# zyddnys/manga-image-translator

Hardware: AMD Instinct MI355X
Metric: pages/sec end-to-end (detect+OCR+inpaint), 2048x1456 (higher is better)
Workload: dtype f32

## Files before the change

include/mit_hip.h:

```cpp
#ifndef MIT_HIP_H
#define MIT_HIP_H

#include <stdint.h>

#ifdef __cplusplus
extern "C" {
#endif

#define MIT_ABI_VERSION 25
#define MIT_MAX_TAPS 64

enum MitAct {
    MIT_ACT_NONE = 0,
    MIT_ACT_RELU = 1,
    MIT_ACT_LEAKY = 2,
    MIT_ACT_SILU = 3,
    MIT_ACT_SIGMOID = 4,
    MIT_ACT_GELU = 5
};
#define MIT_ACT_POST_FIRST 0x100

enum MitPad {
    MIT_PAD_ZERO = 0,
    MIT_PAD_REFLECT = 1
};

typedef struct MitTensorMap {
    float *base;
    int64_t zs1, zs0, bs, ys, xs;
    int64_t nhi;
    int32_t nsplit;
    int32_t _pad;
} MitTensorMap;

typedef struct MitConvGemm {
    const float *a;
    int64_t a_zs1, a_zs0, a_bs, a_ys, a_xs;
    int32_t NB, Hi, Wi, Cin;
    int32_t Ho, Wo, sy, sx;
    int32_t ntaps, pad_mode;
    int8_t tap_dy[MIT_MAX_TAPS];
    int8_t tap_dx[MIT_MAX_TAPS];
    int32_t tap_off[MIT_MAX_TAPS];
    const float *w;
    int64_t w_zs1, w_zs0, ldw;
    int32_t Kw, Nw;
    int32_t N;
    int32_t Z, zdiv;
    MitTensorMap c, pre, post;
    const float *scale, *bias;
    int32_t act;
    float act_alpha;
    const uint16_t *w_split;
    int64_t ws_zs0;
    const int32_t *lut_rows;
    const float *lut1, *lut2;
    int64_t lut_ld;
    int32_t nprod;
    int32_t live_img0;
    const int32_t *live_blocks;
    const int32_t *live_start;
    const float *wino_m;
    int64_t wino_zs;
    int32_t wino_n, wino_th, wino_tw;
    int32_t _pad_wino;
} MitConvGemm;

const char *mit_last_error(void);
int mit_abi_version(void);
const char *mit_source_digest(void);

int mit_device_count(int *count);
int mit_device_name(int device, char *buf, int buflen);

int mit_conv_gemm(const MitConvGemm *desc, void *stream);
int mit_conv_gemm_cfg(const MitConvGemm *desc, int cfg, void *stream);
const char *mit_conv_gemm_config_name(int cfg);
int mit_conv_gemm_plan(const MitConvGemm *desc, int cfg, int32_t *tile, int32_t *nb_run);
const char *mit_conv_gemm_config_kernel(int cfg);

int mit_gemm_split_pack(const float *w_dev, int64_t w_zs, int nz, int Kw, int64_t ldw, uint16_t *out_dev, void *stream);
int mit_gemm_mode_set(int mode);
int mit_gemm_mode_get(void);
int64_t mit_gemm_split_min_tiles(int64_t n);

typedef struct MitPGemm {
    const uint16_t *a_planes;
    int64_t a_zs;
    int64_t lda;
    const uint16_t *w_planes;
    int64_t w_zs;
    int64_t ldw;
// ... 217 lines not shown
                        const int64_t *offsets);
int64_t mit_mask_assign_workspace_bytes(int H, int W);
int mit_mask_assign_lines_dev(uint8_t *mask_dev, int H, int W, const int32_t *boxes_xywh_dev, const double *polys_dev,
                              const double *font_size_dev, int M, int V, double keep_threshold, void *ws_dev, int64_t ws_bytes,
                              int32_t *line_rects_dev, void *stream);
int mit_mask_line_crops_dev(const void *ws_dev, int64_t ws_bytes, int H, int W, const int32_t *jobs_dev, const int64_t *offsets_dev,
                            int n_jobs, int64_t total, uint8_t *out_dev, void *stream);
int mit_merge_mask_list(const uint8_t *cands, const int64_t *scores, int n_cands, const uint8_t *pred_mask, int h, int w,
                        int inpaint_dilate, uint8_t *merged);
int mit_otsu_from_hist(const int32_t *hist, int n, int32_t *thresholds);



typedef struct MitXposTables {
    const float *cos_t, *sin_t, *scale_t, *iscale_t;
    int32_t imax, pmax;
} MitXposTables;

typedef struct MitLinear {
    const float *w, *scale, *bias;
    int64_t ldw;
    int32_t K, N, Kp, Np;
    const uint16_t *w_split;
} MitLinear;

typedef struct MitOcrDecoderLayer {
    const float *ln1_w, *ln1_b, *ln2_w, *ln2_b, *ln3_w, *ln3_b;
    MitLinear qkv;
    MitLinear out;
    MitLinear q2;
    MitLinear out2;
    MitLinear ff1, ff2;
} MitOcrDecoderLayer;

typedef struct MitOcr48Decoder {
    MitOcrDecoderLayer layers[5];
    const float *embd;
    MitLinear pred1;
    MitLinear pred;
    MitLinear color1;
    MitLinear color_heads;
    MitXposTables xpos;
    int32_t dict_size, _pad;
} MitOcr48Decoder;

typedef struct MitOcr48DecodeArgs {
    int32_t N, L;
    const float *mem_k;
    const float *mem_v;
    const int32_t *mem_len;
    int32_t max_seq_length;
    int32_t start_tok, end_tok, max_finished, suppress_eos;
    void *workspace;
    int64_t workspace_bytes;
    int32_t *res_tok;
    int32_t *res_len;
    float *res_prob;
    int32_t *res_row;
    float *colors;
    float *trace_logits;
    int32_t *trace_hist;
    int32_t steps_run;
} MitOcr48DecodeArgs;

typedef struct MitWarpLine {
    double minv[9];
    int32_t page, x1, y1, cw, ch, dw, dh, vertical, out_row, _pad;
} MitWarpLine;
int mit_ocr_warp_lines(const uint8_t *pages_dev, int H, int W, const MitWarpLine *lines_dev, int n_lines, uint8_t *out_dev,
                       int Hout, int Wp, void *stream);
int mit_ocr_prep(const uint8_t *lines_dev, float *out_dev, int N, int H, int Wp, void *stream);
int mit_dwconv_nhwc(const float *in_dev, const float *w_dev, const float *scale_dev, const float *bias_dev, float *out_dev,
                    int B, int H, int W, int C, int k, void *stream);
typedef struct MitRaggedSeg {
    int64_t pixel_start, group_start;
    int32_t B, H, W, _pad;
} MitRaggedSeg;
int mit_dwconv_nhwc_ragged(const float *in_dev, const float *w_dev, const float *scale_dev, const float *bias_dev,
                           float *out_dev, const MitRaggedSeg *segs_dev, int nsegs, int64_t total_groups, int C, int k,
                           void *stream);
int mit_dwconv_nhwc_ragged_rows(const float *in_dev, const float *w_dev, const float *scale_dev, const float *bias_dev,
                                float *out_dev, const MitRaggedSeg *segs_dev, int nsegs, int64_t total_groups, int C, int k,
                                int common_H, void *stream);
int mit_layernorm(const float *in_dev, int64_t in_rowstride, const float *w_dev, const float *b_dev, float *out_dev,
                  int64_t out_rowstride, int rows, int D, float eps, void *stream);
int mit_xpos_rotate(const float *in_dev, int64_t in_rs, int64_t in_ts, float *out_dev, int64_t out_rs, int64_t out_ts, int R,
                    int T, int i0, int p0, int downscale, const MitXposTables *tables, void *stream);
int mit_attention(const float *q_dev, int64_t q_rs, int64_t q_ts, const float *k_dev, int64_t k_rs, int64_t k_ts,
                  const float *v_dev, int64_t v_rs, int64_t v_ts, float *out_dev, int64_t o_rs, int64_t o_ts,
                  const int *klen_dev, int R, int Tq, int Tk, int kv_div, void *stream);
int mit_attention_lines_xpos(const float *q_dev, const float *k_dev, const float *v_dev, float *out_dev, int64_t row_stride,
                             const int32_t *lines_dev, const int *klen_dev, int n_lines, int Lmax, int heads, int head_dim,
                             const MitXposTables *tables, void *stream);
int mit_attention_self_rows_set(int on);
int mit_attention_lines_xpos_max_len(int head_dim);
int mit_memory_kv_lines(const float *k_dev, const float *v_dev, int64_t row_stride, float *mem_k_dev, float *mem_v_dev, int64_t line_stride,
                        const int32_t *lines_dev, int n_lines, int first_line, int64_t n_rows, int Lmax, int head_dim,
                        const MitXposTables *tables, void *stream);
int mit_attention_heads(const float *q_dev, int64_t q_rs, int64_t q_ts, const float *k_dev, int64_t k_rs, int64_t k_ts,
                        const float *v_dev, int64_t v_rs, int64_t v_ts, float *out_dev, int64_t o_rs, int64_t o_ts,
                        const int *klen_dev, int R, int Tq, int Tk, int kv_div, int heads, int head_dim, void *stream);
int mit_avgpool_nhwc(const float *in_dev, float *out_dev, int B, int H, int W, int C, int kh, int kw, int sh, int sw, int ph,
                     int pw, void *stream);
int mit_affine_act_nhwc(const float *in_dev, int64_t in_pixstride, const float *scale_dev, const float *bias_dev, float *out_dev,
                        int64_t out_pixstride, int64_t npix, int C, int relu, void *stream);
int mit_u8_to_f32_nhwc4(const uint8_t *in_dev, float *out_dev, int64_t npix, int mode, void *stream);
int mit_sigmoid_inplace(float *x_dev, int64_t n, void *stream);
int mit_gelu_inplace(float *x_dev, int64_t n, void *stream);
int mit_logsoftmax_top5(const float *logits_dev, int64_t ld, int R, int D, int suppress_tok, float *vals_dev, int *idx_dev,
                        void *stream);
int64_t mit_ocr48_decode_workspace_bytes(int N, int T, int dict_size);
int mit_ocr48_decode(const MitOcr48Decoder *dec, MitOcr48DecodeArgs *args, void *stream);
int mit_ocr48_decode_rows_max_set(int rows);


typedef struct MitOcr32Decoder {
    MitOcrDecoderLayer layers[2];
    const float *embd;
    const float *pe;
    MitLinear pred1;
    MitLinear pred;
    MitLinear color1;
    MitLinear color_heads;
    int32_t dict_size, pe_len;
} MitOcr32Decoder;

typedef struct MitOcr32DecodeArgs {
    int32_t N, L;
    const float *mem_k;
    const float *mem_v;
    const int32_t *mem_len;
    int32_t max_seq_length;
    int32_t start_tok, end_tok;
    int32_t max_finished;
    void *workspace;
    int64_t workspace_bytes;
    int32_t *res_tok;
    int32_t *res_len;
    float *res_prob;
    float *colors;
    int32_t *res_src;
    float *trace_logits;
    int32_t *trace_hist;
    int32_t steps_run;
    int32_t form;
} MitOcr32DecodeArgs;

int64_t mit_ocr32_decode_workspace_bytes(int N, int T, int dict_size);
int mit_ocr32_decode(const MitOcr32Decoder *dec, MitOcr32DecodeArgs *args, void *stream);
int mit_ocr32_beam_replay(const float *vals_dev, const int32_t *idx_dev, int steps, MitOcr32DecodeArgs *args, void *stream);

#ifdef __cplusplus
}
#endif
#endif
```

manga_image_translator_amd/csrc/ocr_kernels.hip:

```cpp

#include <hip/hip_runtime.h>
#include <atomic>
#include <math.h>
#include <stdint.h>
#include <stdlib.h>
#include "../../include/mit_hip.h"
#include "common.h"
#include "ocr_kernels.h"
#include "bf16_split.h"
#include "ln_rows8.h"

typedef float f32x4_t __attribute__((ext_vector_type(4)));

typedef float f32x16 __attribute__((ext_vector_type(16)));

namespace {

__device__ __forceinline__ void store_cells(const OcrPlanes &o, const int k8, const int64_t row, const float *v8) {
    mitcg::u32x4 h, m, l;
    mitcg::split8(*reinterpret_cast<const f32x4 *>(v8), *reinterpret_cast<const f32x4 *>(v8 + 4), h, m, l);
    mitcg::u32x4 *dst = reinterpret_cast<mitcg::u32x4 *>(o.p) + (int64_t)k8 * o.ld + row;
    const int64_t plane = (int64_t)o.K8 * o.ld;
    dst[0] = h;
    dst[plane] = m;
// ... 1551 lines not shown
void ocrk_embed(const int *tok, int64_t tok_stride, const float *E, float *out, int R, int D, hipStream_t s) {
    hipLaunchKernelGGL(embed_kernel, dim3(grid_for((int64_t)R * D / 4, 256)), dim3(256), 0, s, tok, tok_stride, E, out, R, D);
}

void ocrk_logsoftmax_top5(const float *logits, int64_t ld, int R, int D, int suppress_tok, float *vals, int *idx,
                          float *logp_out, hipStream_t s) {
    MitProbeScope probe("logsoftmax_top5_kernel", s, 4.0 * (double)R * D + (logp_out ? 4.0 * (double)R * D : 0.0));
    const char *loop_form = getenv("MIT_OCR_TOP5_LOOP");
    if (loop_form && atoi(loop_form))
        hipLaunchKernelGGL(logsoftmax_top5_kernel<0>, dim3(R), dim3(256), 0, s, logits, ld, D, suppress_tok, vals, idx, logp_out);
    else if (D <= 256 * 8)
        hipLaunchKernelGGL(logsoftmax_top5_kernel<8>, dim3(R), dim3(256), 0, s, logits, ld, D, suppress_tok, vals, idx, logp_out);
    else if (D <= 256 * 24)
        hipLaunchKernelGGL(logsoftmax_top5_kernel<24>, dim3(R), dim3(256), 0, s, logits, ld, D, suppress_tok, vals, idx, logp_out);
    else
        hipLaunchKernelGGL(logsoftmax_top5_kernel<0>, dim3(R), dim3(256), 0, s, logits, ld, D, suppress_tok, vals, idx, logp_out);
}

void ocrk_beam_init(const float *vals, const int *idx, int *hist, int hist_ld, float *logp, int N, int start_tok,
                    hipStream_t s, const float *next_E, float *next_out, int next_D) {
    hipLaunchKernelGGL(beam_init_kernel, dim3(N), dim3(64), 0, s, vals, idx, hist, hist_ld, logp, N, start_tok, BeamNextEmbed{next_E, next_out, next_D});
}

void ocrk_beam_step(const float *vals, const int *idx, const int *hist_in, int *hist_out, int hist_ld, const float *logp_in,
                    float *logp_out, int *done, int *res_row, int *res_len, float *res_prob, int *res_tok, int *done_count,
                    int N, int step, int end_tok, int max_finished, hipStream_t s, const float *next_E, float *next_out, int next_D) {
    hipLaunchKernelGGL(beam_step_kernel, dim3(N), dim3(64), 0, s, vals, idx, hist_in, hist_out, hist_ld, logp_in,
                       logp_out, done, res_row, res_len, res_prob, res_tok, done_count, N, step, end_tok, max_finished,
                       BeamNextEmbed{next_E, next_out, next_D});
}

void ocrk_beam_finalize(const int *hist, int hist_ld, const float *logp, int *done, int *res_row, int *res_len,
                        float *res_prob, int *res_tok, int N, int len, hipStream_t s) {
    hipLaunchKernelGGL(beam_finalize_kernel, dim3((N + 63) / 64), dim3(64), 0, s, hist, hist_ld, logp, done, res_row, res_len,
                       res_prob, res_tok, N, len);
}

extern "C" int mit_ocr_prep(const uint8_t *lines_dev, float *out_dev, int N, int H, int Wp, void *stream) {
    if (!lines_dev || !out_dev) return mit_set_error("mit_ocr_prep: null pointer");
    const int64_t npix = (int64_t)N * H * Wp;
    hipLaunchKernelGGL(ocr_prep_kernel, dim3(grid_for(npix, 256)), dim3(256), 0, (hipStream_t)stream, lines_dev,
                       reinterpret_cast<float4 *>(out_dev), npix);
    MIT_CHECK_LAUNCH("mit_ocr_prep");
    return 0;
}

extern "C" int mit_dwconv_nhwc(const float *in_dev, const float *w_dev, const float *scale_dev, const float *bias_dev,
                               float *out_dev, int B, int H, int W, int C, int k, void *stream) {
    if (!in_dev || !w_dev || !scale_dev || !bias_dev || !out_dev) return mit_set_error("mit_dwconv_nhwc: null pointer");
    if ((C & 3) || !(k & 1)) return mit_set_error("mit_dwconv_nhwc: C %% 4 == 0 and odd k required");
    const int64_t total = (int64_t)B * H * W * (C / 4);
    hipLaunchKernelGGL(dwconv_kernel, dim3(grid_for(total, 256)), dim3(256), 0, (hipStream_t)stream, in_dev, w_dev, scale_dev,
                       bias_dev, out_dev, B, H, W, C / 4, k);
    MIT_CHECK_LAUNCH("mit_dwconv_nhwc");
    return 0;
}


extern "C" int mit_dwconv_nhwc_ragged(const float *in_dev, const float *w_dev, const float *scale_dev, const float *bias_dev,
                                      float *out_dev, const MitRaggedSeg *segs_dev, int nsegs, int64_t total_groups, int C, int k,
                                      void *stream) {
    if (!in_dev || !w_dev || !scale_dev || !bias_dev || !out_dev || !segs_dev) return mit_set_error("mit_dwconv_nhwc_ragged: null pointer");
    if ((C & 3) || nsegs <= 0 || total_groups < 0) return mit_set_error("mit_dwconv_nhwc_ragged: bad arguments");
    if (total_groups == 0) return 0;
    const int C4 = C / 4;
    const int64_t items = total_groups * C4;
    const dim3 grid(grid_for(items, 256) * 4 > 65535 ? 65535 : grid_for(items, 256) * 4), block(256);
    hipStream_t s = (hipStream_t)stream;
    const double elems = 4.0 * (double)total_groups * C;
    MitProbeScope probe(k == 7 ? "dwconv_ragged_kernel<7>" : k == 5 ? "dwconv_ragged_kernel<5>" : "dwconv_ragged_kernel<3>", s, 8.0 * elems, 2.0 * k * k * elems);
    switch (k) {
        case 3: hipLaunchKernelGGL(dwconv_ragged_kernel<3>, grid, block, 0, s, in_dev, w_dev, scale_dev, bias_dev, out_dev, segs_dev, nsegs, C4, items); break;
        case 5: hipLaunchKernelGGL(dwconv_ragged_kernel<5>, grid, block, 0, s, in_dev, w_dev, scale_dev, bias_dev, out_dev, segs_dev, nsegs, C4, items); break;
        case 7: hipLaunchKernelGGL(dwconv_ragged_kernel<7>, grid, block, 0, s, in_dev, w_dev, scale_dev, bias_dev, out_dev, segs_dev, nsegs, C4, items); break;
        default: return mit_set_error("mit_dwconv_nhwc_ragged: k must be 3, 5 or 7 (got %d)", k);
    }
    MIT_CHECK_LAUNCH("mit_dwconv_nhwc_ragged");
    return 0;
}

extern "C" int mit_dwconv_nhwc_ragged_rows(const float *in_dev, const float *w_dev, const float *scale_dev, const float *bias_dev,
                                           float *out_dev, const MitRaggedSeg *segs_dev, int nsegs, int64_t total_groups, int C, int k,
                                           int common_H, void *stream) {
    const int yt = (common_H > 0 && common_H % 4 == 0) ? 4 : (common_H > 0 && common_H % 2 == 0) ? 2 : 0;
    const size_t smem = (size_t)k * k * C * sizeof(float);
    if (yt == 0 || smem > 64 * 1024 || (k != 3 && k != 5 && k != 7))
        return mit_dwconv_nhwc_ragged(in_dev, w_dev, scale_dev, bias_dev, out_dev, segs_dev, nsegs, total_groups, C, k, stream);
    if (!in_dev || !w_dev || !scale_dev || !bias_dev || !out_dev || !segs_dev) return mit_set_error("mit_dwconv_nhwc_ragged_rows: null pointer");
    if ((C & 3) || nsegs <= 0 || total_groups < 0 || total_groups % yt) return mit_set_error("mit_dwconv_nhwc_ragged_rows: bad arguments");
    if (total_groups == 0) return 0;
    const int C4 = C / 4;
    const int64_t items = total_groups / yt * C4;
    const dim3 grid(grid_for(items, 256) * 4 > 65535 ? 65535 : grid_for(items, 256) * 4), block(256);
    hipStream_t s = (hipStream_t)stream;
    const double elems = 4.0 * (double)total_groups * C;
    MitProbeScope probe(k == 7 ? "dwconv_ragged_kernel<7>" : k == 5 ? "dwconv_ragged_kernel<5>" : "dwconv_ragged_kernel<3>", s, 8.0 * elems, 2.0 * k * k * elems);
#define MIT_DWR(KK, YY) hipLaunchKernelGGL((dwconv_ragged_rows_kernel<KK, YY>), grid, block, smem, s, in_dev, w_dev, scale_dev, bias_dev, out_dev, segs_dev, nsegs, C4, common_H, items)
    switch (k * 10 + yt) {
        case 34: MIT_DWR(3, 4); break;
        case 32: MIT_DWR(3, 2); break;
        case 54: MIT_DWR(5, 4); break;
        case 52: MIT_DWR(5, 2); break;
        case 74: MIT_DWR(7, 4); break;
        default: MIT_DWR(7, 2); break;
    }
#undef MIT_DWR
    MIT_CHECK_LAUNCH("mit_dwconv_nhwc_ragged_rows");
    return 0;
}

extern "C" int mit_attention_heads(const float *q_dev, int64_t q_rs, int64_t q_ts, const float *k_dev, int64_t k_rs, int64_t k_ts,
                                   const float *v_dev, int64_t v_rs, int64_t v_ts, float *out_dev, int64_t o_rs, int64_t o_ts,
                                   const int *klen_dev, int R, int Tq, int Tk, int kv_div, int heads, int head_dim, void *stream) {
    if (!q_dev || !k_dev || !v_dev || !out_dev) return mit_set_error("mit_attention_heads: null pointer");
    if (R <= 0 || Tq <= 0 || Tk <= 0 || kv_div <= 0) return mit_set_error("mit_attention_heads: empty problem");
    if (Tk > 8192 || R > 65535 || Tq > 65535) return mit_set_error("mit_attention_heads: problem too large");
    if (heads <= 0 || heads > 64 || head_dim <= 0 || (head_dim & 3) || head_dim > 256)
        return mit_set_error("mit_attention_heads: heads in [1, 64], head_dim a multiple of 4 up to 256");
    ocrk_attention(q_dev, q_rs, q_ts, k_dev, k_rs, k_ts, v_dev, v_rs, v_ts, out_dev, o_rs, o_ts, klen_dev, R, Tq, Tk, kv_div,
                   (hipStream_t)stream, heads, head_dim);
    MIT_CHECK_LAUNCH("mit_attention_heads");
    return 0;
}

extern "C" int mit_avgpool_nhwc(const float *in_dev, float *out_dev, int B, int H, int W, int C, int kh, int kw, int sh, int sw,
                                int ph, int pw, void *stream) {
    if (!in_dev || !out_dev) return mit_set_error("mit_avgpool_nhwc: null pointer");
    if ((C & 3) || kh <= 0 || kw <= 0 || sh <= 0 || sw <= 0 || ph < 0 || pw < 0 || 2 * ph > kh || 2 * pw > kw)
        return mit_set_error("mit_avgpool_nhwc: bad geometry (C %% 4 == 0, pad <= kernel / 2)");
    const int Ho = (H + 2 * ph - kh) / sh + 1, Wo = (W + 2 * pw - kw) / sw + 1;
    if (B <= 0 || Ho <= 0 || Wo <= 0) return mit_set_error("mit_avgpool_nhwc: empty output");
    const int64_t total = (int64_t)B * Ho * Wo * (C / 4);
    hipLaunchKernelGGL(avgpool_general_kernel, dim3(grid_for(total, 256)), dim3(256), 0, (hipStream_t)stream, in_dev, out_dev, B, H, W,
                       C / 4, Ho, Wo, kh, kw, sh, sw, ph, pw);
    MIT_CHECK_LAUNCH("mit_avgpool_nhwc");
    return 0;
}

extern "C" int mit_affine_act_nhwc(const float *in_dev, int64_t in_pixstride, const float *scale_dev, const float *bias_dev,
                                   float *out_dev, int64_t out_pixstride, int64_t npix, int C, int relu, void *stream) {
    if (!in_dev || !scale_dev || !bias_dev || !out_dev) return mit_set_error("mit_affine_act_nhwc: null pointer");
    if ((C & 3) || (in_pixstride & 3) || (out_pixstride & 3)) return mit_set_error("mit_affine_act_nhwc: C and pixel strides must be multiples of 4");
    if (npix <= 0) return 0;
    hipLaunchKernelGGL(affine_act_kernel, dim3(grid_for(npix * (C / 4), 256)), dim3(256), 0, (hipStream_t)stream, in_dev, in_pixstride,
                       scale_dev, bias_dev, out_dev, out_pixstride, npix, C / 4, relu);
    MIT_CHECK_LAUNCH("mit_affine_act_nhwc");
    return 0;
}

extern "C" int mit_logsoftmax_top5(const float *logits_dev, int64_t ld, int R, int D, int suppress_tok, float *vals_dev, int *idx_dev,
                                   void *stream) {
    if (!logits_dev || !vals_dev || !idx_dev) return mit_set_error("mit_logsoftmax_top5: null pointer");
    if (R <= 0 || D < 5) return mit_set_error("mit_logsoftmax_top5: need R > 0 and D >= 5");
    ocrk_logsoftmax_top5(logits_dev, ld, R, D, suppress_tok, vals_dev, idx_dev, nullptr, (hipStream_t)stream);
    MIT_CHECK_LAUNCH("mit_logsoftmax_top5");
    return 0;
}

extern "C" int mit_u8_to_f32_nhwc4(const uint8_t *in_dev, float *out_dev, int64_t npix, int mode, void *stream) {
    if (!in_dev || !out_dev) return mit_set_error("mit_u8_to_f32_nhwc4: null pointer");
    if (mode < 0 || mode > 2) return mit_set_error("mit_u8_to_f32_nhwc4: bad mode %d", mode);
    if (npix <= 0) return 0;
    hipLaunchKernelGGL(u8_to_f32_kernel, dim3(grid_for(npix, 256)), dim3(256), 0, (hipStream_t)stream, in_dev,
                       reinterpret_cast<float4 *>(out_dev), npix, mode);
    MIT_CHECK_LAUNCH("mit_u8_to_f32_nhwc4");
    return 0;
// ... 115 lines not shown
```

manga_image_translator_amd/lib.py:

```python
from __future__ import annotations

import ctypes as C
from pathlib import Path

MIT_MAX_TAPS = 64
MIT_ABI_VERSION = 25

ACT_NONE, ACT_RELU, ACT_LEAKY, ACT_SILU, ACT_SIGMOID, ACT_GELU = range(6)
ACT_POST_FIRST = 0x100
PAD_ZERO, PAD_REFLECT = 0, 1


class MitTensorMap(C.Structure):
    _fields_ = [
        ("base", C.c_void_p),
        ("zs1", C.c_int64),
        ("zs0", C.c_int64),
        ("bs", C.c_int64),
        ("ys", C.c_int64),
        ("xs", C.c_int64),
        ("nhi", C.c_int64),
        ("nsplit", C.c_int32),
        ("_pad", C.c_int32),
    ]


class MitConvGemm(C.Structure):
    _fields_ = [
        ("a", C.c_void_p),
        ("a_zs1", C.c_int64),
        ("a_zs0", C.c_int64),
        ("a_bs", C.c_int64),
        ("a_ys", C.c_int64),
        ("a_xs", C.c_int64),
        ("NB", C.c_int32),
        ("Hi", C.c_int32),
        ("Wi", C.c_int32),
        ("Cin", C.c_int32),
        ("Ho", C.c_int32),
        ("Wo", C.c_int32),
        ("sy", C.c_int32),
        ("sx", C.c_int32),
        ("ntaps", C.c_int32),
        ("pad_mode", C.c_int32),
        ("tap_dy", C.c_int8 * MIT_MAX_TAPS),
        ("tap_dx", C.c_int8 * MIT_MAX_TAPS),
        ("tap_off", C.c_int32 * MIT_MAX_TAPS),
        ("w", C.c_void_p),
        ("w_zs1", C.c_int64),
        ("w_zs0", C.c_int64),
        ("ldw", C.c_int64),
        ("Kw", C.c_int32),
        ("Nw", C.c_int32),
        ("N", C.c_int32),
        ("Z", C.c_int32),
        ("zdiv", C.c_int32),
        ("c", MitTensorMap),
        ("pre", MitTensorMap),
        ("post", MitTensorMap),
        ("scale", C.c_void_p),
        ("bias", C.c_void_p),
        ("act", C.c_int32),
        ("act_alpha", C.c_float),
        ("w_split", C.c_void_p),
        ("ws_zs0", C.c_int64),
        ("lut_rows", C.c_void_p),
        ("lut1", C.c_void_p),
        ("lut2", C.c_void_p),
        ("lut_ld", C.c_int64),
        ("nprod", C.c_int32),
        ("live_img0", C.c_int32),
        ("live_blocks", C.c_void_p),
        ("live_start", C.c_void_p),
        ("wino_m", C.c_void_p),
        ("wino_zs", C.c_int64),
        ("wino_n", C.c_int32),
        ("wino_th", C.c_int32),
        ("wino_tw", C.c_int32),
        ("_pad_wino", C.c_int32),
    ]


class MitPGemm(C.Structure):
    _fields_ = [
        ("a_planes", C.c_void_p), ("a_zs", C.c_int64), ("lda", C.c_int64),
        ("w_planes", C.c_void_p), ("w_zs", C.c_int64), ("ldw", C.c_int64),
        ("M", C.c_int32), ("N", C.c_int32), ("K", C.c_int32), ("Z", C.c_int32),
        ("c", C.c_void_p), ("ldc", C.c_int64), ("c_zs", C.c_int64),
        ("pre", C.c_void_p), ("ld_pre", C.c_int64), ("pre_zs", C.c_int64),
# ... 116 lines not shown
    "mit_prof_tag_next": (C.c_int, [C.c_double]),
    "mit_prof_read": (C.c_int, [C.POINTER(MitProfStat), C.c_int, C.POINTER(C.c_int)]),
    "mit_prof_dump": (C.c_int, [C.c_char_p]),
    "mit_prof_kernels_read": (C.c_int, [C.POINTER(MitProfKernelStat), C.c_int, C.POINTER(C.c_int)]),
    "mit_wino43_input": (C.c_int, [C.c_void_p, C.c_int64, C.c_int64, C.c_int64, C.c_void_p, C.c_int, C.c_int, C.c_int, C.c_int, C.c_int,
                                   C.c_void_p]),
    "mit_wino43_output": (C.c_int, [C.c_void_p, C.c_void_p, C.c_int64, C.c_int64, C.c_int64, C.c_void_p, C.c_int64, C.c_int64, C.c_int64,
                                    C.c_void_p, C.c_void_p, C.c_int, C.c_int, C.c_int, C.c_int, C.c_int, C.c_float, C.c_void_p]),
    "mit_ocr_warp_lines": (C.c_int, [C.c_void_p, C.c_int, C.c_int, C.c_void_p, C.c_int, C.c_void_p, C.c_int, C.c_int,
                                     C.c_void_p]),
    "mit_fft_cols": (C.c_int, [C.c_void_p, C.c_int64, C.c_int64, C.c_int64, C.c_void_p, C.c_int64, C.c_int64, C.c_int64,
                               C.c_void_p, C.c_int, C.c_int, C.c_int64, C.c_int, C.c_float, C.c_void_p]),
    "mit_rfft_rows_supported": (C.c_int, [C.c_int]),
    "mit_rfft_rows": (C.c_int, [C.c_void_p, C.c_int64, C.c_int64, C.c_int64, C.c_void_p, C.c_int64, C.c_int64, C.c_int64, C.c_int64,
                                C.c_void_p, C.c_int, C.c_int, C.c_int, C.c_int, C.c_float, C.c_void_p]),
    "mit_irfft_rows": (C.c_int, [C.c_void_p, C.c_int64, C.c_int64, C.c_int64, C.c_int64, C.c_void_p, C.c_int64, C.c_int64, C.c_int64,
                                 C.c_void_p, C.c_int64, C.c_int64, C.c_int64, C.c_void_p, C.c_int, C.c_int, C.c_int, C.c_int,
                                 C.c_float, C.c_void_p]),
    "mit_bilateral_u8c3": (C.c_int, [C.c_void_p, C.c_void_p, C.c_int, C.c_int, C.c_int, C.c_int, C.c_int, C.c_void_p, C.c_void_p,
                                     C.c_void_p, C.c_void_p]),
    "mit_mask_dilate_jobs": (C.c_int, [C.c_void_p, C.c_void_p, C.c_int, C.c_void_p, C.c_int, C.c_int, C.c_int, C.c_void_p, C.c_void_p]),
    "mit_binarize_u8": (C.c_int, [C.c_void_p, C.c_int64, C.c_void_p]),
    "mit_densecrf_workspace_bytes": (C.c_int64, [C.c_void_p, C.c_int]),
    "mit_densecrf_refine": (C.c_int, [C.c_void_p, C.c_int, C.c_int, C.c_void_p, C.c_int, C.c_void_p, C.c_void_p, C.c_void_p, C.c_float,
                                      C.c_float, C.c_float, C.c_float, C.c_float, C.c_int, C.c_void_p, C.c_void_p, C.c_int64, C.c_void_p]),
    "mit_ctd_refine_workspace_bytes": (C.c_int64, [C.c_void_p, C.c_int]),
    "mit_ctd_refine_hist": (C.c_int, [C.c_void_p, C.c_void_p, C.c_int, C.c_int, C.c_void_p, C.c_int, C.c_void_p, C.c_void_p, C.c_int64,
                                      C.c_void_p]),
    "mit_ctd_refine_scores": (C.c_int, [C.c_void_p, C.c_void_p, C.c_int, C.c_int, C.c_void_p, C.c_int, C.c_void_p, C.c_void_p, C.c_void_p,
                                        C.c_int64, C.c_void_p]),
    "mit_ctd_refine_merge": (C.c_int, [C.c_void_p, C.c_void_p, C.c_int, C.c_int, C.c_void_p, C.c_int, C.c_void_p, C.c_void_p, C.c_void_p,
                                       C.c_int64, C.c_void_p]),
    "mit_lama_prep": (C.c_int, [C.c_void_p, C.c_void_p, C.c_void_p, C.c_int, C.c_int, C.c_int, C.c_void_p]),
    "mit_lama_prep_padded": (C.c_int, [C.c_void_p, C.c_void_p, C.c_void_p, C.c_int, C.c_int, C.c_int, C.c_int, C.c_int, C.c_void_p]),
    "mit_lama_mpe_index": (C.c_int, [C.c_void_p, C.c_int, C.c_int, C.c_int, C.c_void_p, C.c_void_p, C.c_void_p,
                                     C.c_int, C.c_void_p, C.c_void_p, C.c_void_p, C.c_int, C.c_void_p, C.c_void_p,
                                     C.c_void_p, C.c_void_p]),
    "mit_lama_mpe_add": (C.c_int, [C.c_void_p, C.c_void_p, C.c_void_p, C.c_void_p, C.c_void_p, C.c_void_p,
                                   C.c_void_p, C.c_void_p, C.c_float, C.c_float, C.c_int, C.c_int, C.c_int,
                                   C.c_void_p]),
    "mit_lama_mpe_rows": (C.c_int, [C.c_void_p, C.c_void_p, C.c_void_p, C.c_void_p, C.c_void_p, C.c_void_p, C.c_int, C.c_int, C.c_int, C.c_void_p]),
    "mit_ctd_prep": (C.c_int, [C.c_void_p, C.c_int, C.c_int, C.c_int, C.c_int, C.c_int, C.c_int, C.c_int, C.c_void_p,
                               C.c_void_p, C.c_void_p, C.c_void_p, C.c_void_p, C.c_void_p]),
    "mit_maxpool_nhwc": (C.c_int, [C.c_void_p, C.c_int64, C.c_void_p, C.c_int64, C.c_int, C.c_int, C.c_int, C.c_int,
                                   C.c_int, C.c_void_p]),
    "mit_maxpool2d_nhwc": (C.c_int, [C.c_void_p, C.c_void_p, C.c_int, C.c_int, C.c_int, C.c_int, C.c_int, C.c_int, C.c_int,
                                     C.c_void_p]),
    "mit_avgpool2_nhwc": (C.c_int, [C.c_void_p, C.c_int64, C.c_void_p, C.c_int64, C.c_int, C.c_int, C.c_int, C.c_int,
                                    C.c_void_p]),
    "mit_copy_channels": (C.c_int, [C.c_void_p, C.c_int64, C.c_void_p, C.c_int64, C.c_int64, C.c_int, C.c_void_p]),
    "mit_map_to_u8": (C.c_int, [C.c_void_p, C.c_void_p, C.c_int64, C.c_int, C.c_float, C.c_void_p]),
    "mit_axpy": (C.c_int, [C.c_void_p, C.c_float, C.c_void_p, C.c_void_p, C.c_int64, C.c_void_p]),
    "mit_boxes_from_bitmap": (C.c_int, [C.c_void_p, C.c_void_p, C.c_int, C.c_int, C.c_int, C.c_int, C.c_int, C.c_float, C.c_float,
                                        C.c_float, C.c_float, C.c_int, C.c_void_p, C.c_void_p, C.POINTER(C.c_int)]),
    "mit_boxes_debug_stamps": (C.c_int, [C.c_void_p]),
    "mit_boxes_from_bitmap_dev_workspace_bytes": (C.c_int64, [C.c_int, C.c_int, C.c_int, C.c_int]),
    "mit_boxes_from_bitmap_dev": (C.c_int, [C.c_void_p, C.c_int64, C.c_void_p, C.c_int64, C.c_float, C.c_int, C.c_int, C.c_int, C.c_int, C.c_int, C.c_int, C.c_float, C.c_float,
                                            C.c_float, C.c_float, C.c_int, C.c_void_p, C.c_int64, C.c_void_p, C.c_void_p, C.c_void_p, C.c_void_p, C.c_void_p]),
    "mit_merge_mask_list": (C.c_int, [C.c_void_p, C.c_void_p, C.c_int, C.c_void_p, C.c_int, C.c_int, C.c_int, C.c_void_p]),
    "mit_otsu_from_hist": (C.c_int, [C.c_void_p, C.c_int, C.c_void_p]),
    "mit_find_contours_count": (C.c_int, [C.c_void_p, C.c_int, C.c_int, C.POINTER(C.c_int), C.POINTER(C.c_int64)]),
    "mit_mask_assign_lines": (C.c_int, [C.c_void_p, C.c_int, C.c_int, C.c_void_p, C.c_void_p, C.c_void_p, C.c_int, C.c_int, C.c_double, C.c_void_p,
                                        C.c_int64, C.c_void_p, C.c_int64, C.c_void_p, C.POINTER(C.c_int64), C.POINTER(C.c_int32)]),
    "mit_mask_line_crops": (C.c_int, [C.c_void_p, C.c_int64, C.c_void_p, C.c_void_p, C.c_int, C.c_void_p, C.c_void_p]),
    "mit_mask_assign_workspace_bytes": (C.c_int64, [C.c_int, C.c_int]),
    "mit_mask_assign_lines_dev": (C.c_int, [C.c_void_p, C.c_int, C.c_int, C.c_void_p, C.c_void_p, C.c_void_p, C.c_int, C.c_int, C.c_double,
                                            C.c_void_p, C.c_int64, C.c_void_p, C.c_void_p]),
    "mit_mask_line_crops_dev": (C.c_int, [C.c_void_p, C.c_int64, C.c_int, C.c_int, C.c_void_p, C.c_void_p, C.c_int, C.c_int64, C.c_void_p,
                                          C.c_void_p]),
    "mit_ocr_prep": (C.c_int, [C.c_void_p, C.c_void_p, C.c_int, C.c_int, C.c_int, C.c_void_p]),
    "mit_dwconv_nhwc": (C.c_int, [C.c_void_p, C.c_void_p, C.c_void_p, C.c_void_p, C.c_void_p, C.c_int, C.c_int, C.c_int,
                                  C.c_int, C.c_int, C.c_void_p]),
    "mit_quad_pair_distances": (C.c_int, [C.c_void_p, C.c_int, C.c_void_p, C.c_int, C.c_void_p]),
    "mit_ocr48_decode_rows_max_set": (C.c_int, [C.c_int]),
    "mit_pgemm": (C.c_int, [C.POINTER(MitPGemm), C.c_void_p]),
    "mit_pgemm_tile_name": (C.c_char_p, [C.c_int]),
    "mit_pgemm_supported": (C.c_int, [C.POINTER(MitPGemm)]),
    "mit_split_planes": (C.c_int, [C.c_void_p, C.c_int64, C.c_int, C.c_int, C.c_void_p, C.c_int64, C.c_void_p]),
    "mit_join_planes": (C.c_int, [C.c_void_p, C.c_int64, C.c_int, C.c_int, C.c_void_p, C.c_int64, C.c_void_p]),
    "mit_dwconv_nhwc_ragged": (C.c_int, [C.c_void_p, C.c_void_p, C.c_void_p, C.c_void_p, C.c_void_p, C.c_void_p, C.c_int,
                                         C.c_int64, C.c_int, C.c_int, C.c_void_p]),
    "mit_dwconv_nhwc_ragged_rows": (C.c_int, [C.c_void_p, C.c_void_p, C.c_void_p, C.c_void_p, C.c_void_p, C.c_void_p, C.c_int,
                                              C.c_int64, C.c_int, C.c_int, C.c_int, C.c_void_p]),
    "mit_layernorm": (C.c_int, [C.c_void_p, C.c_int64, C.c_void_p, C.c_void_p, C.c_void_p, C.c_int64, C.c_int, C.c_int,
                                C.c_float, C.c_void_p]),
    "mit_xpos_rotate": (C.c_int, [C.c_void_p, C.c_int64, C.c_int64, C.c_void_p, C.c_int64, C.c_int64, C.c_int, C.c_int,
                                  C.c_int, C.c_int, C.c_int, C.POINTER(MitXposTables), C.c_void_p]),
    "mit_attention": (C.c_int, [C.c_void_p, C.c_int64, C.c_int64, C.c_void_p, C.c_int64, C.c_int64, C.c_void_p, C.c_int64,
                                C.c_int64, C.c_void_p, C.c_int64, C.c_int64, C.c_void_p, C.c_int, C.c_int, C.c_int, C.c_int,
                                C.c_void_p]),
    "mit_attention_lines_xpos_max_len": (C.c_int, [C.c_int]),
    "mit_attention_self_rows_set": (C.c_int, [C.c_int]),
    "mit_attention_lines_xpos": (C.c_int, [C.c_void_p, C.c_void_p, C.c_void_p, C.c_void_p, C.c_int64, C.c_void_p, C.c_void_p, C.c_int, C.c_int,
                                           C.c_int, C.c_int, C.POINTER(MitXposTables), C.c_void_p]),
    "mit_memory_kv_lines": (C.c_int, [C.c_void_p, C.c_void_p, C.c_int64, C.c_void_p, C.c_void_p, C.c_int64, C.c_void_p, C.c_int, C.c_int,
                                      C.c_int64, C.c_int, C.c_int, C.POINTER(MitXposTables), C.c_void_p]),
    "mit_attention_heads": (C.c_int, [C.c_void_p, C.c_int64, C.c_int64, C.c_void_p, C.c_int64, C.c_int64, C.c_void_p, C.c_int64,
                                      C.c_int64, C.c_void_p, C.c_int64, C.c_int64, C.c_void_p, C.c_int, C.c_int, C.c_int, C.c_int,
                                      C.c_int, C.c_int, C.c_void_p]),
    "mit_avgpool_nhwc": (C.c_int, [C.c_void_p, C.c_void_p, C.c_int, C.c_int, C.c_int, C.c_int, C.c_int, C.c_int, C.c_int, C.c_int,
                                   C.c_int, C.c_int, C.c_void_p]),
    "mit_affine_act_nhwc": (C.c_int, [C.c_void_p, C.c_int64, C.c_void_p, C.c_void_p, C.c_void_p, C.c_int64, C.c_int64, C.c_int,
                                      C.c_int, C.c_void_p]),
    "mit_u8_to_f32_nhwc4": (C.c_int, [C.c_void_p, C.c_void_p, C.c_int64, C.c_int, C.c_void_p]),
    "mit_sigmoid_inplace": (C.c_int, [C.c_void_p, C.c_int64, C.c_void_p]),
    "mit_gelu_inplace": (C.c_int, [C.c_void_p, C.c_int64, C.c_void_p]),
    "mit_logsoftmax_top5": (C.c_int, [C.c_void_p, C.c_int64, C.c_int, C.c_int, C.c_int, C.c_void_p, C.c_void_p, C.c_void_p]),
    "mit_ocr48_decode_workspace_bytes": (C.c_int64, [C.c_int, C.c_int, C.c_int]),
    "mit_ocr48_decode": (C.c_int, [C.POINTER(MitOcr48Decoder), C.POINTER(MitOcr48DecodeArgs), C.c_void_p]),
    "mit_ocr32_decode_workspace_bytes": (C.c_int64, [C.c_int, C.c_int, C.c_int]),
    "mit_ocr32_decode": (C.c_int, [C.POINTER(MitOcr32Decoder), C.POINTER(MitOcr32DecodeArgs), C.c_void_p]),
    "mit_ocr32_beam_replay": (C.c_int, [C.c_void_p, C.c_void_p, C.c_int, C.POINTER(MitOcr32DecodeArgs), C.c_void_p]),
    "mit_resize_u8": (C.c_int, [C.c_void_p, C.c_int, C.c_int, C.c_int, C.c_int, C.c_void_p, C.c_int, C.c_int, C.c_int, C.c_void_p, C.c_void_p,
                                C.c_void_p, C.c_void_p, C.c_void_p]),
    "mit_resample_pil_u8": (C.c_int, [C.c_void_p, C.c_int, C.c_int, C.c_int, C.c_int, C.c_void_p, C.c_int, C.c_int, C.c_void_p, C.c_void_p,
                                      C.c_int, C.c_void_p]),
    "mit_select_u8": (C.c_int, [C.c_void_p, C.c_int, C.c_void_p, C.c_void_p, C.c_void_p, C.c_int64, C.c_int, C.c_void_p]),
    "mit_rearrange_squares": (C.c_int, [C.c_void_p, C.c_int, C.c_int, C.c_int, C.c_int, C.c_int, C.c_int, C.c_int, C.c_int, C.c_void_p,
                                        C.c_void_p]),
    "mit_rearrange_stitch": (C.c_int, [C.c_void_p, C.c_int, C.c_int, C.c_int, C.c_int64, C.c_int64, C.c_int64, C.c_int64, C.c_int, C.c_int,
                                       C.c_int, C.c_int, C.c_int, C.c_int, C.c_void_p, C.c_void_p, C.c_void_p, C.c_int, C.c_void_p]),
    "mit_lama_post": (C.c_int, [C.c_void_p, C.c_int64, C.c_void_p, C.c_void_p, C.c_void_p, C.c_int, C.c_int, C.c_int, C.c_int,
                                C.c_void_p]),
    "mit_aot_prep": (C.c_int, [C.c_void_p, C.c_void_p, C.c_void_p, C.c_int, C.c_int, C.c_int, C.c_void_p]),
    "mit_aot_gate": (C.c_int, [C.c_void_p, C.c_int64, C.c_void_p, C.c_int64, C.c_int64, C.c_int, C.c_int, C.c_void_p]),
    "mit_aot_plane_stats_ws": (C.c_int64, [C.c_int, C.c_int, C.c_int]),
    "mit_aot_plane_stats": (C.c_int, [C.c_void_p, C.c_int64, C.c_int64, C.c_int, C.c_int, C.c_int, C.c_void_p, C.c_int64, C.c_void_p,
                                      C.c_void_p, C.c_void_p]),
    "mit_aot_blend": (C.c_int, [C.c_void_p, C.c_int64, C.c_int64, C.c_void_p, C.c_int64, C.c_int64, C.c_void_p, C.c_int64, C.c_int64,
                                C.c_void_p, C.c_void_p, C.c_int, C.c_int, C.c_int, C.c_void_p]),
    "mit_aot_post": (C.c_int, [C.c_void_p, C.c_int64, C.c_void_p, C.c_void_p, C.c_void_p, C.c_void_p, C.c_int, C.c_int, C.c_int, C.c_int,
                               C.c_void_p]),
    "mit_grouped_conv3x3": (C.c_int, [C.c_void_p, C.c_int64, C.c_int64, C.c_int, C.c_int, C.c_int, C.c_int, C.c_int, C.c_int, C.c_int,
                                      C.c_void_p, C.c_void_p, C.c_void_p, C.c_int, C.c_float, C.c_void_p, C.c_int64, C.c_int64, C.c_void_p]),
    "mit_grouped_conv3x3_lds_bytes": (C.c_int64, [C.c_int, C.c_int, C.c_int]),
    "mit_se_squeeze_ws": (C.c_int64, [C.c_int, C.c_int, C.c_int]),
    "mit_se_squeeze": (C.c_int, [C.c_void_p, C.c_int64, C.c_int64, C.c_int, C.c_int, C.c_int, C.c_void_p, C.c_int64, C.c_void_p]),
    "mit_se_excite": (C.c_int, [C.c_void_p, C.c_int, C.c_int, C.c_int, C.c_void_p, C.c_void_p, C.c_void_p, C.c_void_p, C.c_void_p,
                                C.c_void_p]),
    "mit_se_apply": (C.c_int, [C.c_void_p, C.c_int64, C.c_int64, C.c_void_p, C.c_void_p, C.c_int64, C.c_int64, C.c_void_p, C.c_int64,
                               C.c_int64, C.c_int, C.c_int, C.c_int, C.c_int, C.c_void_p]),
    "mit_mc2_ffd_pack": (C.c_int, [C.c_void_p, C.c_int, C.c_int, C.c_int, C.c_int, C.c_float, C.c_void_p, C.c_void_p, C.c_void_p]),
    "mit_mc2_ffd_unpack": (C.c_int, [C.c_void_p, C.c_int, C.c_int, C.c_int, C.c_int, C.c_void_p, C.c_void_p, C.c_int64, C.c_void_p,
                                     C.c_void_p, C.c_void_p]),
    "mit_mc2_gen_in": (C.c_int, [C.c_void_p, C.c_int, C.c_int, C.c_int, C.c_void_p, C.c_int, C.c_int, C.c_void_p]),
    "mit_mc2_post": (C.c_int, [C.c_void_p, C.c_int64, C.c_int, C.c_int, C.c_int, C.c_void_p, C.c_int, C.c_int, C.c_void_p]),
    "mit_layernorm_rows": (C.c_int, [C.c_void_p, C.c_int64, C.c_void_p, C.c_void_p, C.c_void_p, C.c_int64, C.c_int64, C.c_int, C.c_float,
                                     C.c_void_p]),
    "mit_dwconv7_ln_nhwc": (C.c_int, [C.c_void_p, C.c_int64, C.c_void_p, C.c_void_p, C.c_void_p, C.c_void_p, C.c_float, C.c_void_p, C.c_int64,
                                      C.c_int, C.c_int, C.c_int, C.c_int, C.c_void_p]),
    "mit_dwconv7_ln_supported": (C.c_int, [C.c_int]),
}

_lib = None


def lib_path() -> Path:
    return Path(__file__).resolve().parent / "libmit_hip.so"


def _stale(path: Path, want: str) -> bool:
    needle = b"MIT_SOURCE_DIGEST=" + want.encode()
    try:
        with open(path, "rb") as f:
            tail = b""
            while True:
# ... 49 lines not shown
```

Measured before the change: 45.66.

## Add LDS-tiled ragged depthwise conv kernel for k=7 tall line crops

Adds a new depthwise-convolution kernel for ragged OCR line batches. Each block stages a full-height tile of 16 channels into LDS together with the weights, then computes 3x4 output pixels per thread from LDS. The existing rows kernel now routes k=7 cases with line height between 13 and 24 to it. The goal is to cut redundant global loads of overlapping input windows, at the cost of large LDS use per block and a persistent grid-stride schedule.

```diff
diff --git a/include/mit_hip.h b/include/mit_hip.h
--- a/include/mit_hip.h
+++ b/include/mit_hip.h
@@ -7,7 +7,7 @@
 extern "C" {
 #endif
 
-#define MIT_ABI_VERSION 25
+#define MIT_ABI_VERSION 26
 #define MIT_MAX_TAPS 64
 
 enum MitAct {
@@ -391,6 +391,10 @@
 int mit_dwconv_nhwc_ragged_rows(const float *in_dev, const float *w_dev, const float *scale_dev, const float *bias_dev,
                                 float *out_dev, const MitRaggedSeg *segs_dev, int nsegs, int64_t total_groups, int C, int k,
                                 int common_H, void *stream);
+int mit_dwconv_ragged_tiled_supported(int C, int k, int H);
+int mit_dwconv_nhwc_ragged_tiled(const float *in_dev, const float *w_dev, const float *scale_dev, const float *bias_dev,
+                                 float *out_dev, const MitRaggedSeg *segs_dev, int nsegs, int64_t total_groups, int C, int k,
+                                 int common_H, void *stream);
 int mit_layernorm(const float *in_dev, int64_t in_rowstride, const float *w_dev, const float *b_dev, float *out_dev,
                   int64_t out_rowstride, int rows, int D, float eps, void *stream);
 int mit_xpos_rotate(const float *in_dev, int64_t in_rs, int64_t in_ts, float *out_dev, int64_t out_rs, int64_t out_ts, int R,
diff --git a/manga_image_translator_amd/csrc/dwconv_tiled.hip b/manga_image_translator_amd/csrc/dwconv_tiled.hip
--- /dev/null
+++ b/manga_image_translator_amd/csrc/dwconv_tiled.hip
@@ -0,0 +1,178 @@
+#include <hip/hip_runtime.h>
+#include <stdint.h>
+#include "../../include/mit_hip.h"
+#include "common.h"
+
+namespace {
+
+typedef float f32x4_t __attribute__((ext_vector_type(4)));
+
+constexpr int CS = 16;
+constexpr int YT = 3;
+constexpr int XT = 4;
+constexpr int MAX_H = 24;
+constexpr int TILE_PIX = 768;
+constexpr int NB = 15;
+
+inline int tiled_xw(int H) { return (TILE_PIX / H) & ~3; }
+inline int tiled_plane(int H, int k) {
+    const int n = H * (tiled_xw(H) + k - 1);
+    return ((n + 14) / 16) * 16 + 1;
+}
+
+template <int K>
+__global__ __launch_bounds__(256, 2) void dwconv_ragged_tiled_kernel(const float *__restrict__ in, const float *__restrict__ w,
+                                                                      const float *__restrict__ scale, const float *__restrict__ bias,
+                                                                      float *__restrict__ out, const MitRaggedSeg *__restrict__ segs,
+                                                                      int nsegs, int C, int H, int XW, int plane) {
+    constexpr int R = K / 2;
+    extern __shared__ __attribute__((aligned(16))) f32x4_t lds[];
+    f32x4_t *wl = lds + 4 * plane;
+    const int tid = threadIdx.x;
+    const int RS = XW + K - 1;
+    const int nslabs = C / CS;
+    const int XG = XW / XT, YG = (H + YT - 1) / YT;
+    const int nitems = 4 * XG * YG;
+    const int nstage = 4 * RS * H;
+    const float inv_rs = 1.0f / (float)RS;
+
+    int64_t nspatial = 0;
+    for (int s = 0; s < nsegs; ++s) nspatial += (int64_t)segs[s].B * ((segs[s].W + XW - 1) / XW);
+    const int64_t u_end = (nspatial + 7) / 8 * 8 * nslabs;
+    int seg = 0;
+    int64_t seg_first = 0;
+    int slab_in_lds = -1;
+
+    for (int64_t u = blockIdx.x; u < u_end; u += gridDim.x) {
+        const int64_t sp = u / (8 * nslabs) * 8 + (u & 7);
+        const int slab = (int)((u >> 3) % nslabs);
+        if (sp >= nspatial) continue;
+        MitRaggedSeg sg = segs[seg];
+        int xtiles = (sg.W + XW - 1) / XW;
+        while (sp >= seg_first + (int64_t)sg.B * xtiles) {
+            seg_first += (int64_t)sg.B * xtiles;
+            sg = segs[++seg];
+            xtiles = (sg.W + XW - 1) / XW;
+        }
+        const int64_t lt = sp - seg_first;
+        const int b = (int)(lt / xtiles);
+        const int x0 = (int)(lt % xtiles) * XW;
+        const int W = sg.W;
+        const int64_t img = (sg.pixel_start + (int64_t)b * H * W) * C + slab * CS;
+        const float *ib = in + img;
+
+        __syncthreads();
+        if (slab != slab_in_lds) {
+            for (int i = tid; i < K * K * 4; i += 256)
+                wl[i] = *reinterpret_cast<const f32x4_t *>(w + (int64_t)(i >> 2) * C + slab * CS + (i & 3) * 4);
+            slab_in_lds = slab;
+        }
+        for (int base = tid; base < nstage; base += 256 * NB) {
+            f32x4_t r[NB];
+            int dst[NB];
+#pragma unroll
+            for (int j = 0; j < NB; ++j) {
+                const int i = base + j * 256;
+                const int pix = i >> 2, q = i & 3;
+                const int row = (int)(((float)pix + 0.5f) * inv_rs);
+                const int col = pix - row * RS;
+                const int xx = x0 + col - R;
+                dst[j] = i < nstage ? q * plane + pix : -1;
+                r[j] = (i < nstage && xx >= 0 && xx < W) ? *reinterpret_cast<const f32x4_t *>(ib + ((int64_t)row * W + xx) * C + q * 4)
+                                                         : f32x4_t{0.f, 0.f, 0.f, 0.f};
+            }
+#pragma unroll
+            for (int j = 0; j < NB; ++j) asm volatile("" : "+v"(r[j]));
+#pragma unroll
+            for (int j = 0; j < NB; ++j)
+                if (dst[j] >= 0) lds[dst[j]] = r[j];
+        }
+        __syncthreads();
+
+        const int wv = min(XW, W - x0);
+        for (int it = tid; it < nitems; it += 256) {
+            const int q = it & 3;
+            const int g = it >> 2;
+            const int yg = g / XG, xg = g - yg * XG;
+            const int xo = xg * XT, y0 = yg * YT;
+            if (xo >= wv) continue;
+            const f32x4_t *pl = lds + q * plane + xo;
+            f32x4_t acc[YT][XT];
+#pragma unroll
+            for (int oy = 0; oy < YT; ++oy)
+#pragma unroll
+                for (int j = 0; j < XT; ++j) acc[oy][j] = f32x4_t{0.f, 0.f, 0.f, 0.f};
+#pragma unroll
+            for (int dr = 0; dr < YT + K - 1; ++dr) {
+                const int yy = y0 + dr - R;
+                if (yy < 0 || yy >= H) continue;
+                f32x4_t v[K + XT - 1];
+#pragma unroll
+                for (int j = 0; j < K + XT - 1; ++j) v[j] = pl[yy * RS + j];
+#pragma unroll
+                for (int oy = 0; oy < YT; ++oy) {
+                    const int ky = dr - oy;
+                    if (ky < 0 || ky >= K) continue;
+#pragma unroll
+                    for (int kx = 0; kx < K; ++kx) {
+                        const f32x4_t ww = wl[(ky * K + kx) * 4 + q];
+#pragma unroll
+                        for (int j = 0; j < XT; ++j) {
+                            acc[oy][j].x = fmaf(v[j + kx].x, ww.x, acc[oy][j].x);
+                            acc[oy][j].y = fmaf(v[j + kx].y, ww.y, acc[oy][j].y);
+                            acc[oy][j].z = fmaf(v[j + kx].z, ww.z, acc[oy][j].z);
+                            acc[oy][j].w = fmaf(v[j + kx].w, ww.w, acc[oy][j].w);
+                        }
+                    }
+                }
+            }
+            const f32x4_t sc = *reinterpret_cast<const f32x4_t *>(scale + slab * CS + q * 4);
+            const f32x4_t bb = *reinterpret_cast<const f32x4_t *>(bias + slab * CS + q * 4);
+#pragma unroll
+            for (int oy = 0; oy < YT; ++oy) {
+                if (y0 + oy >= H) break;
+                float *ob = out + img + ((int64_t)(y0 + oy) * W + x0 + xo) * C + q * 4;
+#pragma unroll
+                for (int j = 0; j < XT; ++j) {
+                    if (xo + j >= wv) break;
+                    f32x4_t o;
+                    o.x = acc[oy][j].x * sc.x + bb.x; o.y = acc[oy][j].y * sc.y + bb.y; o.z = acc[oy][j].z * sc.z + bb.z; o.w = acc[oy][j].w * sc.w + bb.w;
+                    *reinterpret_cast<f32x4_t *>(ob + (int64_t)j * C) = o;
+                }
+            }
+        }
+    }
+}
+
+}
+
+extern "C" int mit_dwconv_ragged_tiled_supported(int C, int k, int H) {
+    return (C > 0 && C % CS == 0 && (k == 3 || k == 5 || k == 7) && H >= 1 && H <= MAX_H) ? 1 : 0;
+}
+
+extern "C" int mit_dwconv_nhwc_ragged_tiled(const float *in_dev, const float *w_dev, const float *scale_dev, const float *bias_dev,
+                                            float *out_dev, const MitRaggedSeg *segs_dev, int nsegs, int64_t total_groups, int C, int k,
+                                            int common_H, void *stream) {
+    if (!mit_dwconv_ragged_tiled_supported(C, k, common_H))
+        return mit_set_error("mit_dwconv_nhwc_ragged_tiled: needs C %% 16 == 0, k in {3, 5, 7} and 1 <= common_H <= 24 (got C = %d, k = %d, H = %d)", C, k, common_H);
+    if (!in_dev || !w_dev || !scale_dev || !bias_dev || !out_dev || !segs_dev) return mit_set_error("mit_dwconv_nhwc_ragged_tiled: null pointer");
+    if (nsegs <= 0 || total_groups < 0 || total_groups % common_H) return mit_set_error("mit_dwconv_nhwc_ragged_tiled: bad arguments");
+    if (total_groups == 0) return 0;
+    const int XW = tiled_xw(common_H), plane = tiled_plane(common_H, k);
+    const size_t smem = ((size_t)4 * plane + (size_t)k * k * 4) * sizeof(f32x4_t);
+    const int64_t max_work = total_groups / common_H * (C / CS);
+    const int64_t want = (max_work + 7) / 8 * 8;
+    const dim3 grid((unsigned)(want < 4096 ? want : 4096)), block(256);
+    hipStream_t s = (hipStream_t)stream;
+    const double elems = 4.0 * (double)total_groups * C;
+    MitProbeScope probe(k == 7 ? "dwconv_ragged_kernel<7>" : k == 5 ? "dwconv_ragged_kernel<5>" : "dwconv_ragged_kernel<3>", s, 8.0 * elems, 2.0 * k * k * elems);
+#define MIT_DWT(KK) hipLaunchKernelGGL(dwconv_ragged_tiled_kernel<KK>, grid, block, smem, s, in_dev, w_dev, scale_dev, bias_dev, out_dev, segs_dev, nsegs, C, common_H, XW, plane)
+    switch (k) {
+        case 3: MIT_DWT(3); break;
+        case 5: MIT_DWT(5); break;
+        default: MIT_DWT(7); break;
+    }
+#undef MIT_DWT
+    MIT_CHECK_LAUNCH("mit_dwconv_nhwc_ragged_tiled");
+    return 0;
+}
diff --git a/manga_image_translator_amd/csrc/ocr_kernels.hip b/manga_image_translator_amd/csrc/ocr_kernels.hip
--- a/manga_image_translator_amd/csrc/ocr_kernels.hip
+++ b/manga_image_translator_amd/csrc/ocr_kernels.hip
@@ -1657,6 +1657,8 @@
 extern "C" int mit_dwconv_nhwc_ragged_rows(const float *in_dev, const float *w_dev, const float *scale_dev, const float *bias_dev,
                                            float *out_dev, const MitRaggedSeg *segs_dev, int nsegs, int64_t total_groups, int C, int k,
                                            int common_H, void *stream) {
+    if (k == 7 && common_H > 12 && mit_dwconv_ragged_tiled_supported(C, k, common_H))
+        return mit_dwconv_nhwc_ragged_tiled(in_dev, w_dev, scale_dev, bias_dev, out_dev, segs_dev, nsegs, total_groups, C, k, common_H, stream);
     const int yt = (common_H > 0 && common_H % 4 == 0) ? 4 : (common_H > 0 && common_H % 2 == 0) ? 2 : 0;
     const size_t smem = (size_t)k * k * C * sizeof(float);
     if (yt == 0 || smem > 64 * 1024 || (k != 3 && k != 5 && k != 7))
diff --git a/manga_image_translator_amd/lib.py b/manga_image_translator_amd/lib.py
--- a/manga_image_translator_amd/lib.py
+++ b/manga_image_translator_amd/lib.py
@@ -4,7 +4,7 @@
 from pathlib import Path
 
 MIT_MAX_TAPS = 64
-MIT_ABI_VERSION = 25
+MIT_ABI_VERSION = 26
 
 ACT_NONE, ACT_RELU, ACT_LEAKY, ACT_SILU, ACT_SIGMOID, ACT_GELU = range(6)
 ACT_POST_FIRST = 0x100
@@ -287,6 +287,9 @@
                                          C.c_int64, C.c_int, C.c_int, C.c_void_p]),
     "mit_dwconv_nhwc_ragged_rows": (C.c_int, [C.c_void_p, C.c_void_p, C.c_void_p, C.c_void_p, C.c_void_p, C.c_void_p, C.c_int,
                                               C.c_int64, C.c_int, C.c_int, C.c_int, C.c_void_p]),
+    "mit_dwconv_ragged_tiled_supported": (C.c_int, [C.c_int, C.c_int, C.c_int]),
+    "mit_dwconv_nhwc_ragged_tiled": (C.c_int, [C.c_void_p, C.c_void_p, C.c_void_p, C.c_void_p, C.c_void_p, C.c_void_p, C.c_int,
+                                               C.c_int64, C.c_int, C.c_int, C.c_int, C.c_void_p]),
     "mit_layernorm": (C.c_int, [C.c_void_p, C.c_int64, C.c_void_p, C.c_void_p, C.c_void_p, C.c_int64, C.c_int, C.c_int,
                                 C.c_float, C.c_void_p]),
     "mit_xpos_rotate": (C.c_int, [C.c_void_p, C.c_int64, C.c_int64, C.c_void_p, C.c_int64, C.c_int64, C.c_int, C.c_int,
```

Result: no change. 45.69, median of 3 (+0.1%).
